# aslpavel/svgrasterize.py

Hardware: AMD Instinct MI355X
Metric: Mpixels/sec AA coverage+composite (path-pixels/s; whole step: flatten+binning+coverage+composite; planned replay -- a frame with new geometry: value_replan) (higher is better)
Workload: dtype f64 arithmetic, f32 RGBA store; 1 GPU; synthetic 4096 random closed cubic paths @ 4096x4096 (SURVEY 8d generator, splitmix64 0x5F3759DF); edges=783607

## Files before the change

### svgrasterize.py_amd/csrc/svgr_hip.hip

```cpp
#include <hip/hip_runtime.h>

#include <algorithm>
#include <atomic>
#include <cstdarg>
#include <cstddef>
#include <cmath>
#include <cstdio>
#include <cstring>
#include <ctime>
#include <initializer_list>
#include <new>
#include <string>
#include <type_traits>
#include <vector>
#include <memory>
#include <unordered_map>
#include <utility>

#include "../../include/svgr.h"
#include "svgr_core.h"

using namespace svgr;

static std::atomic<unsigned long long> g_n_launches{0};
// ... 493 lines not shown
    for (int k = 0; k < 2 * FL_ENDS; ++k) qe[k] = 0.0;
    constexpr int SEGL_ = 1 << SUB;
    if constexpr (PLACED) {
        int first = seg_ok ? lane_off[(size_t)seg * SEGL_ + sub] : 0;
        int nxt = __shfl_down(first, 1);
        if (sub == SEGL_ - 1) nxt = so1 - so0;
        const int n_plan = seg_ok ? nxt - first : 0;
        const int base_p = so0 + first;
        int n_found = 0;
        if (mode == 1) {
            track(node[0], node[1]);
            track(node[6], node[7]);
            n_found = 1;
            if (n_plan >= 1 && base_p < edge_cap) {
                store_edge(edges, base_p, node[0], node[1], node[6], node[7]);
                edge_path[base_p] = p;
            }
        } else if (mode == 2) {
            track(node[0], node[1]);
            int at = 0;
            n_found = flatten_subtree<1>(node, thr, kMaxFlattenDepth - SUB, [&](double r0_, double c0_, double r1, double c1) {
                track(r1, c1);
                if (at < n_plan && base_p + at < edge_cap) {
                    store_edge(edges, base_p + at, r0_, c0_, r1, c1);
                    edge_path[base_p + at] = p;
                }
                ++at;
            }, ovf);
        }
        if (ovf) atomicOr(&bd->err, 1);
        if (keep && n_found != n_plan) atomicOr(&bd->err, 2);
        if (seg_ok && sub == 0 && so1 > so0) atomicAdd(&bd->shard[(int)((blockIdx.x * (FL_BLOCK / 64) + (threadIdx.x >> 6)) % NSH)].cursor, so1 - so0);
    } else {
    const bool census = !EMIT && seg_cnt != nullptr;
    double rows_x = 0.0, cols_x = 0.0;
    if (mode == 1) {
        cnt = 1;
        track(node[0], node[1]);
        track(node[6], node[7]);
        if (census) { rows_x = fabs(node[6] - node[0]); cols_x = fabs(node[7] - node[1]); }
// ... 388 lines not shown
                    sl.e_begin = e_begin; sl.e_end = e_end; sl.pb_off = off;
                    sl.r0 = out[0]; sl.c0 = out[1]; sl.rows = out[2]; sl.cols = out[3];
                    sl.b0 = pb0; sl.cell_off = cell_off;
                    sl.pad[0] = sl.pad[1] = 0;
                    slabs[at++] = sl;
                }
            }
        }
    }
    if (p < n_paths) {
        ((int4*)bbox)[p] = make_int4(out[0], out[1], out[2], out[3]);
        PathBin pbin;
        pbin.b0 = pb0; pbin.nb = pnb; pbin.pb_off = off; pbin.cell_off = cell_off;
        bins[p] = pbin;
    }
}

__device__ __forceinline__ bool edge_prepare(const double* __restrict__ edges, const int* __restrict__ edge_path,
                                             const int* __restrict__ bbox, int e, EdgeSetup& es, int& p, int& r0) {
    p = edge_path[e];
    const int4 bb = ((const int4*)bbox)[p];
    r0 = bb.x;
    const int rows = bb.z, cols = bb.w;
    if (rows <= 0 || cols <= 0) return false;
    const double o_r = (double)bb.x, o_c = (double)bb.y;
    const double* ed = edges + 4 * (size_t)e;
    double ar = ed[0] - o_r, ac = ed[1] - o_c, br = ed[2] - o_r, bc = ed[3] - o_c;
    es = edge_setup(ar, ac, br, bc, rows);
    if (!es.valid) return false;
    double cmin = ac < bc ? ac : bc;
    if (cmin >= (double)cols + 2.0) return false;
    return true;
}

__device__ __forceinline__ void band_rows(const EdgeSetup& es, int band, int vr0, int r0, int& ya, int& yb) {
    const int b0row = band * TR + vr0 - r0;
    ya = es.y_begin > b0row ? es.y_begin : b0row;
    yb = es.y_end < b0row + TR ? es.y_end : b0row + TR;
}

struct TileEntry {
    int c0, cols;
    int cell0;
    int p;
    int r0, rows;
    int pad[2];
};
// ... 739 lines not shown
    int c = __popc(x);
    if (r >= c) { r -= c; pos = 32; x = (unsigned)(m >> 32); }
#pragma unroll
    for (int w = 16; w >= 1; w >>= 1) {
        const unsigned lo = x & ((1u << w) - 1u);
        c = __popc(lo);
        if (r >= c) { r -= c; pos += w; x >>= w; } else { x = lo; }
    }
    return pos;
}
__global__ __launch_bounds__(TL_BLOCK) void k_tile_lists(const int* __restrict__ band_start, const int* __restrict__ band_item0,
                                                         const TileEntry* __restrict__ entries, unsigned long long* __restrict__ tile_mask,
                                                         int mask_words, int n_ct, int vc0, Owner own, int n_owned,
                                                         int2* __restrict__ tile_info, uint4* __restrict__ pages,
                                                         uint4* __restrict__ items, const CellHdr* __restrict__ cell_hdr, int item_cap, int cell_cap,
                                                         BatchDev* __restrict__ bd, const PathBin* __restrict__ bins, const int* __restrict__ bbox) {
    constexpr int NWV = TL_BLOCK / 64;
    __shared__ int s_base[TL_BLOCK + 1], s_rank[TL_BLOCK];
    __shared__ int s_hist[64], s_cur[64], s_wtot[NWV];
    __shared__ int s_run;
    const int tid = threadIdx.x, lane = tid & 63, wave = tid >> 6;
    const int band = owned_band_at(own, blockIdx.x);
    const int W = mask_words;
    const int ent0 = band_start[band], item_band0 = band_item0[band];
    unsigned long long* const mband = tile_mask + (size_t)band * n_ct * 2 * W;
    auto count_tile = [&](int ct, int& n, int& n2) {
        n = 0; n2 = 0;
        const unsigned long long* mw = mband + (size_t)ct * 2 * W;
        for (int w = 0; w < W; ++w) { n += __popcll(mw[w]); n2 += __popcll(mw[W + w]); }
    };
    auto weight_of = [&](int n, int n2) { const int w = n + n2; return w < 63 ? w : 63; };
    if (tid < 64) s_hist[tid] = 0;
    if (tid == 0) s_run = 0;
    __syncthreads();
    const bool one_chunk = n_ct <= TL_BLOCK;
    int n_keep = 0, n2_keep = 0;
    for (int c0 = 0; c0 < n_ct; c0 += TL_BLOCK) {
        const int ct = c0 + tid;
        if (ct < n_ct) {
            int n, n2;
// ... 72 lines not shown
                const int4 eh = *(const int4*)(entries + ent0 + w * 64 + bit);
                cell = eh.z + tct - (eh.x - vc0) / TC;
            }
            const unsigned cls = ((mw[W + w] >> bit) & 1ull) ? 2u : 1u;
            cell = cell >= 0 && cell < cell_cap ? cell : 0;
            const long long at = (long long)item_band0 + run0 + i;
            const int4 hd = cls == 2u ? *(const int4*)((const char*)(cell_hdr + cell) + 48) : make_int4(0, 0, 0, 0);
            const uint4 it = make_uint4((unsigned)cell | (cls << 30), (unsigned)hd.z, (unsigned)hd.y, 0u);
            if (at < (long long)item_cap) items[at] = it;
            if (r_tile < PAGE_ITEMS) pages[((size_t)s_rank[lo] * n_owned + blockIdx.x) * PAGE_STRIDE + r_tile] = it;
        }
        __syncthreads();
        if (tid == 0) s_run = run0 + total;
        if (ct < n_ct) {
            unsigned long long* mw = mband + (size_t)ct * 2 * W;
            for (int w = 0; w < 2 * W; ++w) mw[w] = 0ull;
        }
        __syncthreads();
    }
}

constexpr int GRAD_MAX_STOPS = 32;
struct GradDev {
    int kind, spread, has_gt, n_stops;
    int excl_enabled, pad0, pad1, pad2;
    double user_m6[6], gt_m6[6];
    double p0[2], vec[2], vv;
    double center[2], radius;
    double fcenter[2], fradius, cd[2], rd, a, frad_rd, frad2, excl_thresh;
    double stop_off[GRAD_MAX_STOPS];
// ... 1963 lines not shown
    void wait_uploads() {
        if (up_pending && up_ev) (void)hipEventSynchronize(up_ev);
        up_pending = false;
        host_keep.clear();
    }
    DevArr<unsigned char> arena;
    size_t arena_bytes = 0, arena_laid = 0, off_pkeys = 0, off_prow = 0, off_scan = 0;
    DevArr<int> edge_path, bbox, band_start, band_count;
    DevArr<PathBin> bins;
    DevArr<TileEntry> entries;
    DevArr<double> edges;
    DevArr<CellHdr> cell_hdr;
    DevArr<unsigned char> work_block;
    DevArr<int2> cell_plan;
    bool add_places = false;
    void invalidate_work() { masks_zeroed = false; arena_zeroed = false; slabs_current = false; }
    DevArr<TileAdd> adds;
    DevArr<uint4> items;
    DevArr<int2> tile_info;
    DevArr<uint4> pages;
    DevArr<int> band_item0;
    AddShards add_shards{};
    int64_t n_adds = 0;
    bool count_adds_only = false;
    bool adds_roomy = false;
    bool fl_scan = false;
    bool late_scan = false;
    bool census_bbox = false;
    bool deterministic = false;
    int size_adds(const int* need, int n_shards) {
        if (int rc = layout_adds(need, n_shards)) return rc;
// ... 15 lines not shown
    DevArr<int> pair_idx;
    DevArr<Slab> slabs;
    DevArr<int> slab_at;
    bool slab_at_valid = false;
    bool slabs_current = false;
    bool slab_order_late = false;
    struct SlabsMade {
        const void *slabs, *bbox, *bins, *slab_at;
        int64_t n_slabs, n_paths;
        int vp[4];
        bool operator==(const SlabsMade& o) const {
            return slabs == o.slabs && bbox == o.bbox && bins == o.bins && slab_at == o.slab_at && n_slabs == o.n_slabs && n_paths == o.n_paths &&
                   vp[0] == o.vp[0] && vp[1] == o.vp[1] && vp[2] == o.vp[2] && vp[3] == o.vp[3];
        }
    } slabs_made{};
    bool slab_order_pending = false;
    std::vector<int> slab_at_host;
    int64_t n_slabs = 0;
    DevArr<int> seg_cnt, seg_off;
    int fl_sub = FL_SUB;
    DevArr<int> lane_off;
    DevArr<int> path_seg0;
    DevArr<int> seg_list;
    int64_t n_seg_list = -1;
    DevArr<int> path_list;
    int64_t n_path_list = 0;
    DevArr<unsigned long long> tile_mask;
    int mask_words = 1;
    bool masks_zeroed = false;
    DevArr<long long> layer_off;
    std::vector<long long> host_layer_off;
    bool geometry_fresh = false;
    bool geometry_current = false;
    bool arena_zeroed = false;
    int64_t n_edges_live = 0;
    int64_t n_edges = 0, n_pb = 0, n_bsegs = 0, n_cells = 0, n_entries = 0;
    int n_bands = 0;
    BatchDev host_bd{};
    EdgeShards shards{};
    std::vector<int> host_bbox;
    bool host_bbox_stale = false;
    bool defer_bbox = false;
    std::vector<TimedEvents> events;
    std::vector<hipEvent_t> event_pool;

    int n_ctiles() const { return (vp[3] + TC - 1) / TC; }
    int size_tile_lists(int owned_bands) {
        const size_t nt = (size_t)std::max(n_bands, 1) * (size_t)std::max(n_ctiles(), 1);
        if (int rc = tile_info.ensure(nt)) return rc;
        if (int rc = pages.ensure((size_t)std::max(owned_bands, 1) * (size_t)std::max(n_ctiles(), 1) * PAGE_STRIDE)) return rc;
        if (int rc = band_item0.ensure((size_t)n_bands + 1)) return rc;
        return items.ensure((size_t)std::max<int64_t>(n_cells, 1));
    }
    size_t mask_bytes() const { return sizeof(unsigned long long) * 2 * (size_t)mask_words * (size_t)n_bands * (size_t)n_ctiles(); }
    int size_masks(int64_t longest) {
        mask_words = (int)std::max<int64_t>((longest + 63) / 64, 1);
        masks_zeroed = false;
        return tile_mask.ensure(mask_bytes() / sizeof(unsigned long long) + 1);
    }
    bool census_set = false;
    BatchDev* bd() const { return (BatchDev*)arena.p + (census_set ? 1 : 0); }
    unsigned long long* pkeys() const { return (unsigned long long*)(arena.p + off_pkeys); }
    unsigned* prow() const { return (unsigned*)(arena.p + off_prow); }
    unsigned long long* scan_state() const { return (unsigned long long*)(arena.p + off_scan); }

    int layout_arena() {
        off_pkeys = 2 * sizeof(BatchDev);
        off_prow = off_pkeys + sizeof(unsigned long long) * 4 * (size_t)n_paths;
        off_scan = (off_prow + sizeof(unsigned) * 2 * (size_t)n_paths + 7) & ~(size_t)7;
        arena_bytes = off_scan + sizeof(unsigned long long) * (((size_t)n_segs << 6) / FL_BLOCK + 2);
        arena_bytes = (arena_bytes + 255) & ~(size_t)255;
        const unsigned char* const before = arena.p;
// ... 15 lines not shown
    int vp[4] = {0, 0, 0, 0};
    int64_t n_segs = 0, n_paths = 0;
    int mask_words = 1;
    AddShards add_shards{};
    int64_t n_adds = 0;
    bool adds_roomy = false;
    DevArr<int> edge_path, band_start, band_count, pair_idx, slab_at, seg_cnt, seg_off, lane_off, band_item0;
    DevArr<TileEntry> entries;
    DevArr<double> edges;
    DevArr<CellHdr> cell_hdr;
    DevArr<unsigned char> work_block;
    DevArr<int2> cell_plan, tile_info;
    DevArr<TileAdd> adds;
    DevArr<uint4> items, pages;
    DevArr<Slab> slabs;
    DevArr<unsigned long long> tile_mask;
};
#define SVGR_SPARE_ARRAYS(X) X(edge_path) X(band_start) X(band_count) X(pair_idx) X(slab_at) X(seg_cnt) X(seg_off) X(lane_off) X(band_item0) \
    X(entries) X(edges) X(cell_hdr) X(work_block) X(cell_plan) X(tile_info) X(adds) X(items) X(pages) X(slabs) X(tile_mask)
static void spare_stash(svgr_batch* b) {
    svgr_ctx* c = b->ctx;
    if (!b->sized || !b->has_vp || b->own.world > 1 || b->n_segs <= 4096 || !b->edges.p || !b->cell_plan.p || getenv("SVGR_NO_SPARE")) return;
    if (!c->spare) c->spare = new (std::nothrow) WorkSpare();
    if (!c->spare) return;
    WorkSpare& w = *c->spare;
    for (int k = 0; k < 4; ++k) w.vp[k] = b->sized_vp[k];
    w.n_segs = b->n_segs; w.n_paths = b->n_paths; w.mask_words = b->mask_words; w.add_shards = b->add_shards; w.n_adds = b->n_adds; w.adds_roomy = b->adds_roomy;
#define X(a) w.a = std::move(b->a);
    SVGR_SPARE_ARRAYS(X)
#undef X
}
static bool spare_adopt(svgr_batch* b) {
    svgr_ctx* c = b->ctx;
    WorkSpare* w = c->spare;
    if (!w || !w->edges.p || b->sized || !b->has_vp || b->own.world > 1 || b->n_segs <= 4096) return false;
    for (int k = 0; k < 4; ++k) if (w->vp[k] != b->vp[k]) return false;
    if (b->n_segs * 2 < w->n_segs || b->n_segs > w->n_segs + w->n_segs / 2 || b->n_paths * 2 < w->n_paths || b->n_paths > w->n_paths + w->n_paths / 2) return false;
    if (w->slab_at.cap && w->slab_at.cap < (size_t)b->n_paths) return false;
#define X(a) b->a = std::move(w->a);
    SVGR_SPARE_ARRAYS(X)
#undef X
    b->mask_words = w->mask_words; b->add_shards = w->add_shards; b->n_adds = w->n_adds; b->adds_roomy = w->adds_roomy;
    b->n_bands = (b->vp[2] + TR - 1) / TR;
    b->masks_zeroed = false;
    b->slab_at_valid = false; b->slabs_current = false;
    b->sized = true;
    for (int k = 0; k < 4; ++k) b->sized_vp[k] = b->vp[k];
    return true;
}

static inline dim3 grid1(size_t n, int block = 256) { return dim3((unsigned)((n + block - 1) / block)); }
static inline int cap_i32(size_t n) { return (int)std::min<size_t>(n, 0x7fffffff); }

static int choose_fl_sub(const svgr_batch* b, int n_items) {
    const size_t waves32 = ((size_t)std::max(n_items, 1) << 5) / 64, slots = (size_t)b->ctx->n_cu * 4 * 6;
    return waves32 * 2 <= slots ? 6 : 5;
}
static int run_geometry(svgr_batch* b, int upto, bool use_vp) {
    hipStream_t st = b->ctx->stream;
    const int ns = (int)b->n_segs, np = (int)b->n_paths;
    if (!b->arena_zeroed) HIPCHK(hipMemsetAsync(b->arena.p, 0, b->arena_bytes, st));
    b->arena_zeroed = false;
    const bool listed = use_vp && b->own.world > 1 && b->n_seg_list >= 0;
    const int n_items = listed ? (int)b->n_seg_list : ns;
    if (upto == 1) b->fl_sub = choose_fl_sub(b, n_items);
    const int fl_sub = b->fl_sub;
    const dim3 fgrid = grid1((size_t)std::max(n_items, 1) << fl_sub, FL_BLOCK);
    const int* seg_list = listed ? (const int*)b->seg_list.p : (const int*)nullptr;
    const int* plist = listed ? (const int*)b->path_list.p : (const int*)nullptr;
    const int np_walk = listed ? (int)b->n_path_list : np;
    const unsigned* prow = nullptr;
    if (use_vp && b->own.world > 1 && ns > 0 && !listed) {
        SVGR_LAUNCH(k_path_rows, grid1((size_t)ns), dim3(256), 0, st, (const double*)b->segs.p, (const uint8_t*)b->seg_kind.p,
                           (const int*)b->seg_path.p, (const double*)b->path_m6.p, ns, b->prow());
        prow = b->prow();
    }
    const int n_bands_vp = use_vp ? (b->vp[2] + TR - 1) / TR : 0;
// ... 6 lines not shown
        }
        if (ns > 0) {
            auto launch_cnt = [&](auto kern) {
                SVGR_LAUNCH(kern, fgrid, dim3(FL_BLOCK), 0, st, (const double*)b->segs.p,
                                   (const uint8_t*)b->seg_kind.p, (const int*)b->seg_path.p, (const double*)b->path_m6.p, ns,
                                   b->thr, (double*)nullptr, (int*)nullptr, b->shards, b->pkeys(), b->bd(), b->own, b->vp[0],
                                   n_bands_vp, prow, seg_list, n_items, upto == 1 ? b->seg_cnt.p : (int*)nullptr, (const int*)nullptr,
                                   use_vp ? b->vp[3] : 0 ,
                                   upto == 1 ? b->lane_off.p : (int*)nullptr, (int*)nullptr, (unsigned long long*)nullptr);
            };
            if (fl_sub == 6) launch_cnt(k_flatten<false, false, 6>); else launch_cnt(k_flatten<false, false, 5>);
        }
        if (upto == 1 && !b->late_scan)
            SVGR_LAUNCH(k_seg_scan, dim3(1), dim3(1024), 0, st, (const int*)b->seg_cnt.p, ns, b->seg_off.p);
        if (upto == 0 || (upto == 1 && b->census_bbox)) {
            b->slabs_current = false;
            SVGR_LAUNCH(k_path_bbox, grid1((size_t)std::max(np_walk, 1), 64), dim3(64), 0, st, (const unsigned long long*)b->pkeys(),
                               np_walk, use_vp ? 1 : 0, b->vp[0], b->vp[1], b->vp[2], b->vp[3], b->bbox.p, b->bins.p, b->bd(), 1, plist,
                               (Slab*)nullptr, 0, b->own, (const int*)nullptr, (const int*)nullptr, 0, (const int*)nullptr);
        }
        return 0;
    }
    if (ns > 0) {
        const bool lane_places = !b->safe_path;
        auto launch_fl = [&](auto kern, int* places) {
            SVGR_LAUNCH(kern, fgrid, dim3(FL_BLOCK), 0, st, (const double*)b->segs.p,
                               (const uint8_t*)b->seg_kind.p, (const int*)b->seg_path.p, (const double*)b->path_m6.p, ns, b->thr,
                               b->edges.p, b->edge_path.p, b->shards, b->pkeys(), b->bd(), b->own, b->vp[0],
                               n_bands_vp, prow, seg_list, n_items, (int*)nullptr, (const int*)b->seg_off.p,
                               cap_i32(std::min(b->edge_path.cap, b->edges.cap / 4)), places, (int*)nullptr, (unsigned long long*)nullptr);
        };
        const bool placed_fl = lane_places && b->lane_off.p && b->lane_off.cap >= ((size_t)ns << fl_sub);
        if (b->fl_scan) {
            auto launch_scan = [&](auto kern) {
                SVGR_LAUNCH(kern, fgrid, dim3(FL_BLOCK), 0, st, (const double*)b->segs.p,
                                   (const uint8_t*)b->seg_kind.p, (const int*)b->seg_path.p, (const double*)b->path_m6.p, ns, b->thr,
                                   b->edges.p, b->edge_path.p, b->shards, b->pkeys(), b->bd(), b->own, b->vp[0],
                                   n_bands_vp, prow, seg_list, n_items, b->seg_cnt.p, (const int*)nullptr,
                                   cap_i32(std::min(b->edge_path.cap, b->edges.cap / 4)), b->lane_off.p, b->seg_off.p, b->scan_state());
            };
            if (fl_sub == 6) launch_scan(k_flatten<true, false, 6, true>); else launch_scan(k_flatten<true, false, 5, true>);
        } else if (fl_sub == 6) {
            if (placed_fl) launch_fl(k_flatten<true, true, 6>, b->lane_off.p); else launch_fl(k_flatten<true, false, 6>, (int*)nullptr);
// ... 8 lines not shown
    const bool keep_slabs = slabs_for_plan && placed && b->slabs_current && b->slabs_made == slabs_now;
    if (!keep_slabs) {
        SVGR_LAUNCH(k_path_bbox, grid1((size_t)std::max(np_walk, 1), 64), dim3(64), 0, st, (const unsigned long long*)b->pkeys(), np_walk,
                           use_vp ? 1 : 0, b->vp[0], b->vp[1], b->vp[2], b->vp[3], b->bbox.p, b->bins.p, b->bd(), b->planned ? 0 : 1, plist,
                           upto >= 3 ? b->slabs.p : (Slab*)nullptr, (int)std::min<int64_t>(cap_i32(b->slabs.cap), b->n_slabs) , b->own,
                           (const int*)b->path_seg0.p, (const int*)b->seg_off.p,
                           cap_i32(std::min(b->edge_path.cap, b->edges.cap / 4)),
                           upto >= 4 && b->planned && b->slab_at_valid ? (const int*)b->slab_at.p : (const int*)nullptr);
        b->slabs_current = slabs_for_plan && !b->slab_order_late;
        b->slab_order_late = false;
        b->slabs_made = slabs_now;
    }
    if (upto == 2) return 0;
    const int owned = count_owned_bands(b->own, b->n_bands);
    const bool clear_in_be = owned > 0 && !keep_lists && upto >= 4 && !b->masks_zeroed && b->tile_mask.p && b->own.world <= 1;
    if (owned > 0 && !keep_lists)
        SVGR_LAUNCH(k_band_entries, dim3(owned), dim3(BE_BLOCK), 0, st, (const PathBin*)b->bins.p, np_walk, plist,
                           (const int*)b->bbox.p, b->band_start.p, b->band_count.p, b->band_item0.p, b->entries.p,
                           b->pair_idx.p, cap_i32(std::min(b->entries.cap, b->pair_idx.cap)),
                           upto >= 4 ? cap_i32(b->items.cap) : 0x7fffffff, b->vp[1], b->bd(), b->own,
                           upto >= 4 && b->planned && use_vp && !b->safe_path ? 1 : 0,
                           clear_in_be ? b->tile_mask.p : (unsigned long long*)nullptr, b->n_ctiles() * 2 * b->mask_words);
    if (clear_in_be) b->masks_zeroed = true;
    if (upto == 3) return 0;
    if (!b->masks_zeroed && b->tile_mask.p) {
        HIPCHK(hipMemsetAsync(b->tile_mask.p, 0, b->mask_bytes(), st));
        b->masks_zeroed = true;
    }
    unsigned long long* pb_dbg = nullptr;
#ifdef SVGR_DBG_PB_STAMP
    {
        static unsigned long long* buf = nullptr;
        if (!buf) { (void)hipMalloc((void**)&buf, 8 * 8 * 8192); (void)hipMemset(buf, 0, 8 * 8 * 8192); }
        pb_dbg = buf;
    }
#endif
    if (b->n_slabs > 0) {
        b->masks_zeroed = false;
        auto launch_pb = [&](auto kern) {
            SVGR_LAUNCH(kern, dim3((unsigned)b->n_slabs), dim3(PB_THREADS), 0, st, (const Slab*)b->slabs.p, (const double*)b->edges.p,
                               (const int*)b->pair_idx.p, (const double*)b->path_paint.p, (const uint8_t*)b->path_rule.p,
                               b->n_groups > 0 ? (const int*)b->path_group.p : (const int*)nullptr,
                               b->n_grads > 0 ? (const int*)b->path_grad.p : (const int*)nullptr, b->vp[0], b->vp[1], b->n_ctiles(), b->mask_words,
                               b->tile_mask.p, b->cell_hdr.p, cap_i32(std::min(b->cell_hdr.cap, b->cell_plan.cap)), b->add_shards,
                               b->count_adds_only ? (TileAdd*)nullptr : b->adds.p, b->cell_plan.p, b->bd(), b->own, b->planned ? 0 : 1,
                               b->deterministic ? 1 : 0, pb_dbg, keep_slabs ? (const unsigned long long*)b->pkeys() : (const unsigned long long*)nullptr,
                               (const int*)b->bbox.p, (const PathBin*)b->bins.p, np, b->vp[2], b->vp[3]);
        };
        const bool bounded = !placed && !b->count_adds_only && b->adds.p && b->adds_roomy && !b->safe_path && !getenv("SVGR_SAFE_PATH");
        if (getenv("SVGR_DBG_PLAN"))
            fprintf(stderr, "[geometry] k_path_build<%d>%s, %lld slabs, slab table %s\n", placed ? 1 : bounded ? 2 : 0,
                    b->count_adds_only ? " measuring" : "", (long long)b->n_slabs, keep_slabs ? "kept" : "written");
        if (placed) launch_pb(k_path_build<1>); else if (bounded) launch_pb(k_path_build<2>); else launch_pb(k_path_build<0>);
#ifdef SVGR_DBG_PB_STAMP
        if (pb_dbg && b->planned && !b->count_adds_only) {
            static int n_dump = 0;
            if (++n_dump == 20) {
                HIPCHK(hipStreamSynchronize(st));
                const size_t n = (size_t)std::min<int64_t>(b->n_slabs, 8192);
                std::vector<unsigned long long> h(8 * n);
                HIPCHK(hipMemcpy(h.data(), pb_dbg, sizeof(unsigned long long) * h.size(), hipMemcpyDeviceToHost));
                double ph[5] = {0, 0, 0, 0, 0}, rows_ = 0;
                unsigned long long lo = ~0ull, hi = 0;
                for (size_t i = 0; i < n; ++i) {
                    for (int q = 0; q < 5; ++q) ph[q] += (double)(h[8 * i + q + 1] - h[8 * i + q]);
                    rows_ += (double)h[8 * i + 6];
                    lo = std::min(lo, h[8 * i]); hi = std::max(hi, h[8 * i + 3]);
                }
                double s_rec = 0, s_edges = 0;
                for (size_t i = 0; i < n; ++i) { s_rec += (double)(h[8 * i + 7] - h[8 * i]); s_edges += (double)(h[8 * i + 5] - h[8 * i + 7]); }
                fprintf(stderr, "[pb stamp] %zu slabs, mean us: stage %.2f (slab record %.2f, edges landed +%.2f)  passA %.2f  walk %.2f | rows/slab %.0f | span %.1f us\n", n,
                        ph[0] / n / 100, s_rec / n / 100, s_edges / n / 100, ph[1] / n / 100, ph[2] / n / 100, rows_ / n, (double)(hi - lo) / 100);
                if (const char* f = getenv("SVGR_DBG_PB_DUMP")) { if (FILE* fp = fopen(f, "wb")) { fwrite(h.data(), 8, h.size(), fp); fclose(fp); } }
            }
        }
#endif
    }
    if (owned > 0 && b->n_ctiles() > 0) {
        SVGR_LAUNCH(k_tile_lists, dim3(owned), dim3(TL_BLOCK), 0, st, (const int*)b->band_start.p, (const int*)b->band_item0.p,
                           (const TileEntry*)b->entries.p, b->tile_mask.p, b->mask_words, b->n_ctiles(), b->vp[1], b->own, owned,
                           b->tile_info.p, b->pages.p, b->items.p, (const CellHdr*)b->cell_hdr.p, cap_i32(b->items.cap), cap_i32(b->cell_hdr.cap), b->bd(),
                           keep_lists ? (const PathBin*)b->bins.p : (const PathBin*)nullptr, (const int*)b->bbox.p);
        b->masks_zeroed = true;
    }
    return 0;
}

static int eval_dev_err(int e, int* capacity_bits) {
    if (capacity_bits) { *capacity_bits = e & (2 | 4 | 8 | 32 | 64); e &= ~(2 | 4 | 8 | 32 | 64); }
    if (e & 1) return fail(SVGR_E_OVERFLOW, "flatten depth cap (%d) hit: non-finite or absurd control points", kMaxFlattenDepth);
    if (e & 16) return fail(SVGR_E_INVALID, "path extent beyond +-1e9 pixels or non-finite");
    if (e & (2 | 4 | 8 | 32 | 64)) return fail(SVGR_E_OVERFLOW, "work buffer capacity exceeded (err bits %d): call svgr_batch_plan again", e);
    return 0;
}
static int issue_readback(svgr_batch* b, bool with_bboxes, void* staging = nullptr) {
    void* bd_dst = staging ? staging : (void*)&b->host_bd;
    HIPCHK(hipMemcpyAsync(bd_dst, b->bd(), sizeof(BatchDev), hipMemcpyDeviceToHost, b->ctx->stream));
    if (with_bboxes && !(b->defer_bbox && staging)) {
        b->host_bbox.resize(4 * (size_t)b->n_paths);
// ... 568 lines not shown

int svgr_batch_set_transforms(svgr_batch* b, const double* path_m6) {
    if (!b || !path_m6) return fail(SVGR_E_INVALID, "bad arguments");
    for (int64_t i = 0; i < 6 * b->n_paths; ++i)
        if (!std::isfinite(path_m6[i])) return fail(SVGR_E_INVALID, "non-finite transform");
    HIPCHK(enter_ctx(b->ctx));
    const size_t mbytes = sizeof(double) * 6 * (size_t)b->n_paths;
    if (void* hs = upload_stage(b->ctx, mbytes)) {
        memcpy(hs, path_m6, mbytes);
        HIPCHK(upload_staged(b->ctx, b->path_m6.p, mbytes));
    } else {
        b->wait_uploads();
        HIPCHK(hipMemcpyAsync(b->path_m6.p, b->keep(path_m6, mbytes), mbytes, hipMemcpyHostToDevice, b->ctx->stream));
        HIPCHK(b->note_upload(b->ctx->stream));
    }
    b->planned = false; b->slab_at_valid = false; b->slabs_current = false; b->slab_order_pending = false;
    return 0;
}

int svgr_batch_set_bands(svgr_batch* b, int rank, int world, int strip_bands) {
    if (!b || world <= 0 || rank < 0 || rank >= world || strip_bands <= 0) return fail(SVGR_E_INVALID, "bad band selection");
    b->own = Owner{rank, world, strip_bands};
    b->planned = false; b->slab_at_valid = false; b->slabs_current = false; b->slab_order_pending = false;
    b->sized = false;
    b->n_seg_list = -1;
    return 0;
}

int svgr_batch_set_groups(svgr_batch* b, const int32_t* path_group, int64_t n_groups, const int32_t* group_clip_src,
                          const double* group_opacity) {
    return abi_guard("svgr_batch_set_groups", [&]() -> int {
        if (!b) return fail(SVGR_E_INVALID, "batch is NULL");
        if (n_groups == 0) { b->n_groups = 0; b->geometry_fresh = false; b->geometry_current = false; return 0; }
        if (n_groups < 0 || n_groups > b->n_paths || !path_group || !group_clip_src || !group_opacity)
            return fail(SVGR_E_INVALID, "svgr_batch_set_groups: bad arguments");
        std::vector<int64_t> first((size_t)n_groups, -1), last((size_t)n_groups, -1);
        for (int64_t p = 0; p < b->n_paths; ++p) {
            const int g = path_group[p];
// ... 199 lines not shown
    return 1;
}
static int plan_slab_order(svgr_batch* b);
static int plan_speculative(svgr_batch* b) {
    for (int again = 1; again >= 0; --again) {
        const int is = spec_issue(b, nullptr, again != 0);
        if (is < 0) return is;
        if (is == 0) continue;
        HIPCHK(hipStreamSynchronize(b->ctx->stream));
        HIPCHK(hipGetLastError());
        const int fin = spec_finish(b);
        if (fin > 0 && b->n_segs > 4096) {
            if (int rc = plan_slab_order(b)) return rc;
        }
        if (fin != 0) return fin;
        b->planned = false; b->slabs_current = false;
    }
    return 0;
}

static int build_seg_list(svgr_batch* b) {
    hipStream_t st = b->ctx->stream;
    const int ns = (int)b->n_segs;
    if (int rc = b->seg_list.ensure((size_t)ns)) return rc;
    HIPCHK(hipMemsetAsync(b->arena.p, 0, b->arena_bytes, st));
    b->arena_zeroed = false;
    SVGR_LAUNCH(k_path_rows, grid1((size_t)ns), dim3(256), 0, st, (const double*)b->segs.p, (const uint8_t*)b->seg_kind.p,
                       (const int*)b->seg_path.p, (const double*)b->path_m6.p, ns, b->prow());
    SVGR_LAUNCH(k_seg_select, grid1((size_t)ns), dim3(256), 0, st, (const int*)b->seg_path.p, ns, (const unsigned*)b->prow(), b->own,
                       b->vp[0], (b->vp[2] + TR - 1) / TR, b->seg_list.p, &b->bd()->edge_spare);
    int n = 0;
// ... 48 lines not shown
        std::vector<char> issued((size_t)n, 0);
        std::vector<size_t> stage_off((size_t)n, 0);
        std::map<svgr_ctx*, size_t> stage_need;
        for (int64_t i = 0; i < n; ++i) {
            size_t& need = stage_need[batches[i]->ctx];
            stage_off[(size_t)i] = need;
            need += (sizeof(BatchDev) + 16 * (size_t)batches[i]->n_paths + 255) & ~(size_t)255;
        }
        for (auto& kv : stage_need) {
            HIPCHK(enter_ctx(kv.first));
            if (int rc = ensure_pinned(kv.first, kv.second)) return rc;
        }
        for (int64_t i = 0; i < n; ++i) {
            svgr_batch* b = batches[i];
            HIPCHK(enter_ctx(b->ctx));
            b->planned = false; b->slab_at_valid = false; b->slabs_current = false; b->slab_order_pending = false;
            b->geometry_fresh = false; b->geometry_current = false;
            const int is = no_spec ? 0 : spec_issue(b, (char*)b->ctx->pinned + stage_off[(size_t)i]);
            if (is < 0) return is;
            issued[(size_t)i] = (char)is;
        }
        for (int64_t i = 0; i < n; ++i)
            if (issued[(size_t)i]) {
                HIPCHK(enter_ctx(batches[i]->ctx));
                HIPCHK(hipStreamSynchronize(batches[i]->ctx->stream));
                HIPCHK(hipGetLastError());
                take_readback(batches[i], (const char*)batches[i]->ctx->pinned + stage_off[(size_t)i]);
            }
        for (int64_t i = 0; i < n; ++i) {
            svgr_batch* b = batches[i];
            int done = 0;
            if (issued[(size_t)i]) {
                done = spec_finish(b);
                if (done < 0) return done;
                if (done > 0 && b->n_segs > 4096)
                    if (int rc = plan_slab_order(b)) return rc;
            }
            if (!done)
                if (int rc = batch_plan_impl(b, issued[(size_t)i] != 0)) return rc;
        }
        return 0;
    });
}

static int plan_slab_order(svgr_batch* b) {
    b->slab_at_valid = false; b->slabs_current = false;
    b->slab_order_late = false;
    if (getenv("SVGR_SAFE_PATH")) return 0;
    const size_t np = (size_t)b->n_paths;
    if (int rc = ensure_host_bbox(b)) return rc;
    if (np == 0 || b->host_bbox.size() < 4 * np || b->n_slabs <= 0 || b->vp[2] <= 0) return 0;
    std::vector<int> n_sl(np, 0), order;
    std::vector<float> w(np, 0.f);
    order.reserve(np);
    long long total = 0;
    for (size_t p = 0; p < np; ++p) {
        const int r0 = b->host_bbox[4 * p], c0 = b->host_bbox[4 * p + 1], rows = b->host_bbox[4 * p + 2], cols = b->host_bbox[4 * p + 3];
        if (rows <= 0 || cols <= 0) continue;
        const int pb0 = (r0 - b->vp[0]) / TR, pnb = (r0 + rows - 1 - b->vp[0]) / TR - pb0 + 1;
        int ct0, pnct;
        path_ctiles(c0, cols, b->vp[1], ct0, pnct);
// ... 96 lines not shown
        diff[(size_t)b1 + 1] -= 1;
    }
    int longest = 0, run = 0;
    for (int k = 0; k < b->n_bands; ++k) { run += diff[(size_t)k]; longest = std::max(longest, run); }
    {
        double guess = 1.1 * (2.0 * (double)rows_x + (double)cols_x) + 14.0 * (double)b->n_cells + 65536.0;
        if (const char* sk = getenv("SVGR_TWO_PASS_SHRINK")) guess /= std::max(atof(sk), 1.0);
        if (guess > (double)(1ll << 29)) return 0;
        int need[NSH];
        for (int k = 0; k < NSH; ++k) need[k] = (int)(guess * 1.15 / NSH) + 8192;
        if ((rc = b->layout_adds(need, NSH))) return rc;
        b->adds_roomy = true;
    }
    b->mask_words = (int)std::max<int64_t>(((int64_t)std::max(longest, 1) + 63) / 64, 1);
    b->masks_zeroed = false;
    {
        const size_t n_e = (size_t)std::max<int64_t>(b->n_edges, 1), n_c = (size_t)std::max<int64_t>(b->n_cells, 1);
        const size_t n_pairs = (size_t)std::max<int64_t>(b->n_pb, 1), n_bd = (size_t)b->n_bands + 1;
        const size_t n_tiles = (size_t)std::max(b->n_bands, 1) * (size_t)std::max(b->n_ctiles(), 1);
        const size_t owned = (size_t)std::max(count_owned_bands(b->own, b->n_bands), 1);
        auto layout = [&](Carver& c) {
            c.take(b->edges, n_e * 4);
            c.take(b->edge_path, n_e);
            c.take(b->band_start, n_bd);
            c.take(b->band_count, n_bd);
            c.take(b->band_item0, n_bd);
            c.take(b->cell_hdr, n_c + 1);
            c.take(b->cell_plan, n_c + 1);
            c.take(b->slabs, (size_t)std::max<int64_t>(b->n_slabs, 1));
            c.take(b->entries, n_pairs);
            c.take(b->pair_idx, n_pairs);
            c.take(b->tile_mask, b->mask_bytes() / sizeof(unsigned long long) + 1);
            c.take(b->tile_info, n_tiles);
            c.take(b->pages, owned * (size_t)std::max(b->n_ctiles(), 1) * PAGE_STRIDE);
            c.take(b->items, n_c);
            c.take(b->adds, (size_t)std::max<int64_t>(b->n_adds, 1));
        };
        Carver sizing;
        layout(sizing);
        b->edges.release(); b->edge_path.release(); b->band_start.release(); b->band_count.release(); b->band_item0.release();
        b->cell_hdr.release(); b->cell_plan.release(); b->slabs.release(); b->entries.release(); b->pair_idx.release();
        b->tile_mask.release(); b->tile_info.release(); b->pages.release(); b->items.release(); b->adds.release();
        b->work_block.release();
        if ((rc = b->work_block.ensure(sizing.at))) return rc;
        Carver carve;
        carve.base = b->work_block.p;
        layout(carve);
    }
    const double t_3 = now_ms();
    if ((rc = run_geometry(b, 4, true))) return rc;
    if ((rc = issue_readback(b, staging == nullptr, staging))) return rc;
    if (getenv("SVGR_DBG_PLAN"))
        fprintf(stderr, "[plan] two passes, ms: pass 1 issued %.3f, drained %.3f, buffers sized %.3f, pass 2 issued %.3f | edges %lld, rows crossed %lld, columns %lld, pairs %lld, cells %lld, slabs %lld, add slots %lld, longest band list %d\n",
                t_1 - t_0, t_2 - t_1, t_3 - t_2, now_ms() - t_3, n_edges, rows_x, cols_x, (long long)b->n_pb, (long long)b->n_cells, (long long)b->n_slabs, (long long)b->n_adds, longest);
    return 1;
}
static int two_pass_finish(svgr_batch* b, const void* staging) {
// ... 21 lines not shown

static int plan_two_pass(svgr_batch* b) {
    const int is = two_pass_issue(b, nullptr);
    if (is <= 0) return is;
    HIPCHK(hipStreamSynchronize(b->ctx->stream));
    const int fin = two_pass_finish(b, nullptr);
    if (fin <= 0) return fin;
    if (int rc = plan_slab_order(b)) return rc;
    return 1;
}

static int batch_plan_impl(svgr_batch* b, bool skip_speculative) {
    if (!b) return fail(SVGR_E_INVALID, "batch is NULL");
    HIPCHK(enter_ctx(b->ctx));
    b->defer_bbox = false;
    b->planned = false; b->slab_at_valid = false; b->slabs_current = false; b->slab_order_pending = false;
    b->geometry_fresh = false; b->geometry_current = false;
    {
        const bool no_spec = getenv("SVGR_NO_SPECULATIVE_PLAN") != nullptr;
        const int sp = no_spec || skip_speculative ? 0 : plan_speculative(b);
        if (sp < 0) return sp;
        if (sp > 0) return 0;
    }
    {
        const int tp = plan_two_pass(b);
        if (tp < 0) return tp;
        if (tp > 0) return 0;
        b->planned = false; b->slab_at_valid = false; b->slabs_current = false; b->slab_order_pending = false;
        b->geometry_fresh = false; b->geometry_current = false;
    }
    if (int rc = b->layout_arena()) return rc;
    if (!b->has_vp) {
        if (int rc = run_geometry(b, 0, false)) return rc;
        if (int rc = check_dev_err(b)) return rc;
        if (b->host_bd.n_nonempty > 0) {
            long long r0 = (long long)UNION_BIAS - (long long)b->host_bd.umin_r, c0 = (long long)UNION_BIAS - (long long)b->host_bd.umin_c;
            long long ur = (long long)b->host_bd.umax_r - UNION_BIAS - r0, uc = (long long)b->host_bd.umax_c - UNION_BIAS - c0;
            if (ur * uc > (1ll << 31) || ur > (1 << 24) || uc > (1 << 24))
                return fail(SVGR_E_INVALID, "unclipped extent of %lldx%lld pixels is too large; pass a viewport", ur, uc);
            b->vp[0] = (int)r0; b->vp[1] = (int)c0; b->vp[2] = (int)ur; b->vp[3] = (int)uc;
        } else {
            b->vp[0] = b->vp[1] = 0; b->vp[2] = b->vp[3] = 0;
        }
// ... 423 lines not shown
}

static int batch_draw_impl(svgr_batch* b, svgr_buf* out, int out_kind, unsigned flags) {
    if (!b || !out) return fail(SVGR_E_INVALID, "bad arguments");
    HIPCHK(enter_ctx(b->ctx));
    hipStream_t st = b->ctx->stream;
    b->defer_bbox = false;
    if (!b->planned) {
        const bool canvas = out_kind == SVGR_OUT_CANVAS_F32 || out_kind == SVGR_OUT_CANVAS_F64;
        const bool fast = canvas && b->has_vp && b->own.world <= 1 && b->n_segs > 0 && !(flags & (SVGR_RENDER_TIMED | SVGR_RENDER_DETERMINISTIC)) &&
                          getenv("SVGR_NO_SPECULATIVE_PLAN") == nullptr && getenv("SVGR_SAFE_PATH") == nullptr;
        int issued = 0;
        if (fast) {
            const size_t stage_bytes = sizeof(BatchDev) + 16 * (size_t)b->n_paths + 256;
            if (int rc = ensure_pinned(b->ctx, stage_bytes)) return rc;
            b->slab_at_valid = false; b->slabs_current = false; b->slab_order_pending = false;
            b->geometry_fresh = false; b->geometry_current = false;
            b->defer_bbox = true;
            int is = spec_issue(b, b->ctx->pinned, true);
            b->defer_bbox = is > 0;
            if (is == 0) is = spec_issue(b, b->ctx->pinned, false);
            if (is < 0) return is;
            if (is > 0) issued = 1;
            else {
                is = two_pass_issue(b, b->ctx->pinned);
                if (is < 0) return is;
                if (is > 0) issued = 2;
            }
        }
        if (issued) {
            b->planned = true; b->geometry_fresh = true; b->geometry_current = true;
            int rc = batch_render_impl(b, out, out_kind, flags, nullptr);
            b->planned = false; b->slabs_current = false; b->geometry_fresh = false; b->geometry_current = false;
            hipError_t e = hipStreamSynchronize(st);
            if (rc) return rc;
            HIPCHK(e);
            int fin;
            if (issued == 1) { take_readback(b, b->ctx->pinned); HIPCHK(hipGetLastError()); fin = spec_finish(b); }
            else fin = two_pass_finish(b, b->ctx->pinned);
            b->defer_bbox = false;
            if (fin < 0) return fin;
            if (fin > 0) {
                b->geometry_fresh = false;
                b->slab_order_pending = b->n_segs > 4096;
                return 0;
            }
            b->planned = false; b->slab_at_valid = false; b->slabs_current = false; b->slab_order_pending = false;
        }
        if (int rc = batch_plan_impl(b, issued == 1)) return rc;
    }
    if (int rc = batch_render_impl(b, out, out_kind, flags, nullptr)) return rc;
    HIPCHK(hipStreamSynchronize(st));
    return check_dev_err(b, nullptr, false);
}
int svgr_batch_draw(svgr_batch* b, svgr_buf* out, int out_kind, unsigned flags) {
    return abi_guard("svgr_batch_draw", [&]() { return batch_draw_impl(b, out, out_kind, flags); });
}

int svgr_batch_timings(svgr_batch* b, int* n_renders, double* ms_total, double* ms_geometry, double* ms_tile) {
    if (!b) return fail(SVGR_E_INVALID, "batch is NULL");
    HIPCHK(enter_ctx(b->ctx));
    HIPCHK(hipStreamSynchronize(b->ctx->stream));
// ... 1767 lines not shown
```

Before: 811,400 Mpixels/s.

## Reuse tile lists when tile masks are unchanged across planned replays

```diff
diff --git a/svgrasterize.py_amd/csrc/svgr_hip.hip b/svgrasterize.py_amd/csrc/svgr_hip.hip
--- a/svgrasterize.py_amd/csrc/svgr_hip.hip
+++ b/svgrasterize.py_amd/csrc/svgr_hip.hip
@@ -531,7 +531,7 @@
             n_found = 1;
             if (n_plan >= 1 && base_p < edge_cap) {
                 store_edge(edges, base_p, node[0], node[1], node[6], node[7]);
-                edge_path[base_p] = p;
+                if (edge_path) edge_path[base_p] = p;
             }
         } else if (mode == 2) {
             track(node[0], node[1]);
@@ -540,7 +540,7 @@
                 track(r1, c1);
                 if (at < n_plan && base_p + at < edge_cap) {
                     store_edge(edges, base_p + at, r0_, c0_, r1, c1);
-                    edge_path[base_p + at] = p;
+                    if (edge_path) edge_path[base_p + at] = p;
                 }
                 ++at;
             }, ovf);
@@ -959,23 +959,6 @@
         pbin.b0 = pb0; pbin.nb = pnb; pbin.pb_off = off; pbin.cell_off = cell_off;
         bins[p] = pbin;
     }
-}
-
-__device__ __forceinline__ bool edge_prepare(const double* __restrict__ edges, const int* __restrict__ edge_path,
-                                             const int* __restrict__ bbox, int e, EdgeSetup& es, int& p, int& r0) {
-    p = edge_path[e];
-    const int4 bb = ((const int4*)bbox)[p];
-    r0 = bb.x;
-    const int rows = bb.z, cols = bb.w;
-    if (rows <= 0 || cols <= 0) return false;
-    const double o_r = (double)bb.x, o_c = (double)bb.y;
-    const double* ed = edges + 4 * (size_t)e;
-    double ar = ed[0] - o_r, ac = ed[1] - o_c, br = ed[2] - o_r, bc = ed[3] - o_c;
-    es = edge_setup(ar, ac, br, bc, rows);
-    if (!es.valid) return false;
-    double cmin = ac < bc ? ac : bc;
-    if (cmin >= (double)cols + 2.0) return false;
-    return true;
 }
 
 __device__ __forceinline__ void band_rows(const EdgeSetup& es, int band, int vr0, int r0, int& ya, int& yb) {
@@ -1745,7 +1728,8 @@
                                                          int mask_words, int n_ct, int vc0, Owner own, int n_owned,
                                                          int2* __restrict__ tile_info, uint4* __restrict__ pages,
                                                          uint4* __restrict__ items, const CellHdr* __restrict__ cell_hdr, int item_cap, int cell_cap,
-                                                         BatchDev* __restrict__ bd, const PathBin* __restrict__ bins, const int* __restrict__ bbox) {
+                                                         BatchDev* __restrict__ bd, const PathBin* __restrict__ bins, const int* __restrict__ bbox,
+                                                         unsigned long long* __restrict__ tile_mask_kept, int kept) {
     constexpr int NWV = TL_BLOCK / 64;
     __shared__ int s_base[TL_BLOCK + 1], s_rank[TL_BLOCK];
     __shared__ int s_hist[64], s_cur[64], s_wtot[NWV];
@@ -1753,8 +1737,44 @@
     const int tid = threadIdx.x, lane = tid & 63, wave = tid >> 6;
     const int band = owned_band_at(own, blockIdx.x);
     const int W = mask_words;
+    unsigned long long* const mband = tile_mask + (size_t)band * n_ct * 2 * W;
+    unsigned long long* const kband = tile_mask_kept ? tile_mask_kept + (size_t)band * n_ct * 2 * W : nullptr;
+    if (kept) {
+        __shared__ int s_wdiff[NWV];
+        auto any_differs = [&](bool d) {
+            const bool wd = __ballot(d) != 0ull;
+            if (lane == 0) s_wdiff[wave] = wd ? 1 : 0;
+            __syncthreads();
+            int a = 0;
+#pragma unroll
+            for (int w = 0; w < NWV; ++w) a |= s_wdiff[w];
+            return a != 0;
+        };
+        unsigned long long diff = 0ull;
+        if (W == 1 && n_ct <= TL_BLOCK) {
+            ulonglong2 m = make_ulonglong2(0ull, 0ull), k = m;
+            if (tid < n_ct) { m = ((const ulonglong2*)mband)[tid]; k = ((const ulonglong2*)kband)[tid]; }
+            diff = (m.x ^ k.x) | (m.y ^ k.y);
+            if (!any_differs(diff != 0ull)) {
+                if ((m.x | m.y) != 0ull) ((ulonglong2*)mband)[tid] = make_ulonglong2(0ull, 0ull);
+                return;
+            }
+        } else {
+            for (int ct = tid; ct < n_ct; ct += TL_BLOCK) {
+                const unsigned long long* mw = mband + (size_t)ct * 2 * W;
+                const unsigned long long* kw = kband + (size_t)ct * 2 * W;
+                for (int w = 0; w < 2 * W; ++w) diff |= mw[w] ^ kw[w];
+            }
+            if (!any_differs(diff != 0ull)) {
+                for (int ct = tid; ct < n_ct; ct += TL_BLOCK) {
+                    unsigned long long* mw = mband + (size_t)ct * 2 * W;
+                    for (int w = 0; w < 2 * W; ++w) mw[w] = 0ull;
+                }
+                return;
+            }
+        }
+    }
     const int ent0 = band_start[band], item_band0 = band_item0[band];
-    unsigned long long* const mband = tile_mask + (size_t)band * n_ct * 2 * W;
     auto count_tile = [&](int ct, int& n, int& n2) {
         n = 0; n2 = 0;
         const unsigned long long* mw = mband + (size_t)ct * 2 * W;
@@ -1857,6 +1877,10 @@
         if (tid == 0) s_run = run0 + total;
         if (ct < n_ct) {
             unsigned long long* mw = mband + (size_t)ct * 2 * W;
+            if (kband) {
+                unsigned long long* kw = kband + (size_t)ct * 2 * W;
+                for (int w = 0; w < 2 * W; ++w) kw[w] = mw[w];
+            }
             for (int w = 0; w < 2 * W; ++w) mw[w] = 0ull;
         }
         __syncthreads();
@@ -3850,7 +3874,7 @@
     DevArr<unsigned char> work_block;
     DevArr<int2> cell_plan;
     bool add_places = false;
-    void invalidate_work() { masks_zeroed = false; arena_zeroed = false; slabs_current = false; }
+    void invalidate_work() { masks_zeroed = false; arena_zeroed = false; slabs_current = false; lists_current = false; }
     DevArr<TileAdd> adds;
     DevArr<uint4> items;
     DevArr<int2> tile_info;
@@ -3896,6 +3920,22 @@
                    vp[0] == o.vp[0] && vp[1] == o.vp[1] && vp[2] == o.vp[2] && vp[3] == o.vp[3];
         }
     } slabs_made{};
+    bool lists_current = false;
+    struct ListsMade {
+        const void *items, *pages, *tile_info, *entries, *bins, *bbox, *cell_hdr, *cell_plan, *tile_mask, *tile_mask_kept;
+        size_t items_cap, pages_cap, tile_info_cap, entries_cap, bins_cap, bbox_cap, cell_hdr_cap, cell_plan_cap, tile_mask_cap, tile_mask_kept_cap;
+        int n_ctiles, mask_words, owned;
+        int vp[4];
+        bool operator==(const ListsMade& o) const {
+            return items == o.items && pages == o.pages && tile_info == o.tile_info && entries == o.entries && bins == o.bins && bbox == o.bbox &&
+                   cell_hdr == o.cell_hdr && cell_plan == o.cell_plan && tile_mask == o.tile_mask && tile_mask_kept == o.tile_mask_kept &&
+                   items_cap == o.items_cap && pages_cap == o.pages_cap && tile_info_cap == o.tile_info_cap && entries_cap == o.entries_cap &&
+                   bins_cap == o.bins_cap && bbox_cap == o.bbox_cap && cell_hdr_cap == o.cell_hdr_cap && cell_plan_cap == o.cell_plan_cap &&
+                   tile_mask_cap == o.tile_mask_cap && tile_mask_kept_cap == o.tile_mask_kept_cap && n_ctiles == o.n_ctiles &&
+                   mask_words == o.mask_words && owned == o.owned && vp[0] == o.vp[0] && vp[1] == o.vp[1] && vp[2] == o.vp[2] && vp[3] == o.vp[3];
+        }
+    } lists_made{};
+    unsigned long long stale_word = 0ull;
     bool slab_order_pending = false;
     std::vector<int> slab_at_host;
     int64_t n_slabs = 0;
@@ -3908,6 +3948,7 @@
     DevArr<int> path_list;
     int64_t n_path_list = 0;
     DevArr<unsigned long long> tile_mask;
+    DevArr<unsigned long long> tile_mask_kept;
     int mask_words = 1;
     bool masks_zeroed = false;
     DevArr<long long> layer_off;
@@ -3938,6 +3979,8 @@
     int size_masks(int64_t longest) {
         mask_words = (int)std::max<int64_t>((longest + 63) / 64, 1);
         masks_zeroed = false;
+        lists_current = false;
+        if (int rc = tile_mask_kept.ensure(mask_bytes() / sizeof(unsigned long long) + 1)) return rc;
         return tile_mask.ensure(mask_bytes() / sizeof(unsigned long long) + 1);
     }
     bool census_set = false;
@@ -3983,10 +4026,10 @@
     DevArr<TileAdd> adds;
     DevArr<uint4> items, pages;
     DevArr<Slab> slabs;
-    DevArr<unsigned long long> tile_mask;
+    DevArr<unsigned long long> tile_mask, tile_mask_kept;
 };
 #define SVGR_SPARE_ARRAYS(X) X(edge_path) X(band_start) X(band_count) X(pair_idx) X(slab_at) X(seg_cnt) X(seg_off) X(lane_off) X(band_item0) \
-    X(entries) X(edges) X(cell_hdr) X(work_block) X(cell_plan) X(tile_info) X(adds) X(items) X(pages) X(slabs) X(tile_mask)
+    X(entries) X(edges) X(cell_hdr) X(work_block) X(cell_plan) X(tile_info) X(adds) X(items) X(pages) X(slabs) X(tile_mask) X(tile_mask_kept)
 static void spare_stash(svgr_batch* b) {
     svgr_ctx* c = b->ctx;
     if (!b->sized || !b->has_vp || b->own.world > 1 || b->n_segs <= 4096 || !b->edges.p || !b->cell_plan.p || getenv("SVGR_NO_SPARE")) return;
@@ -4012,7 +4055,7 @@
     b->mask_words = w->mask_words; b->add_shards = w->add_shards; b->n_adds = w->n_adds; b->adds_roomy = w->adds_roomy;
     b->n_bands = (b->vp[2] + TR - 1) / TR;
     b->masks_zeroed = false;
-    b->slab_at_valid = false; b->slabs_current = false;
+    b->slab_at_valid = false; b->slabs_current = false; b->lists_current = false;
     b->sized = true;
     for (int k = 0; k < 4; ++k) b->sized_vp[k] = b->vp[k];
     return true;
@@ -4030,6 +4073,7 @@
     const int ns = (int)b->n_segs, np = (int)b->n_paths;
     if (!b->arena_zeroed) HIPCHK(hipMemsetAsync(b->arena.p, 0, b->arena_bytes, st));
     b->arena_zeroed = false;
+    if (upto < 4) b->lists_current = false;
     const bool listed = use_vp && b->own.world > 1 && b->n_seg_list >= 0;
     const int n_items = listed ? (int)b->n_seg_list : ns;
     if (upto == 1) b->fl_sub = choose_fl_sub(b, n_items);
@@ -4066,7 +4110,7 @@
         if (upto == 1 && !b->late_scan)
             SVGR_LAUNCH(k_seg_scan, dim3(1), dim3(1024), 0, st, (const int*)b->seg_cnt.p, ns, b->seg_off.p);
         if (upto == 0 || (upto == 1 && b->census_bbox)) {
-            b->slabs_current = false;
+            b->slabs_current = false; b->lists_current = false;
             SVGR_LAUNCH(k_path_bbox, grid1((size_t)std::max(np_walk, 1), 64), dim3(64), 0, st, (const unsigned long long*)b->pkeys(),
                                np_walk, use_vp ? 1 : 0, b->vp[0], b->vp[1], b->vp[2], b->vp[3], b->bbox.p, b->bins.p, b->bd(), 1, plist,
                                (Slab*)nullptr, 0, b->own, (const int*)nullptr, (const int*)nullptr, 0, (const int*)nullptr);
@@ -4075,10 +4119,11 @@
     }
     if (ns > 0) {
         const bool lane_places = !b->safe_path;
+        const bool keep_edge_path = b->planned && lane_places && b->lane_off.p && b->lane_off.cap >= ((size_t)ns << fl_sub) && !b->fl_scan;
         auto launch_fl = [&](auto kern, int* places) {
             SVGR_LAUNCH(kern, fgrid, dim3(FL_BLOCK), 0, st, (const double*)b->segs.p,
                                (const uint8_t*)b->seg_kind.p, (const int*)b->seg_path.p, (const double*)b->path_m6.p, ns, b->thr,
-                               b->edges.p, b->edge_path.p, b->shards, b->pkeys(), b->bd(), b->own, b->vp[0],
+                               b->edges.p, keep_edge_path ? (int*)nullptr : b->edge_path.p, b->shards, b->pkeys(), b->bd(), b->own, b->vp[0],
                                n_bands_vp, prow, seg_list, n_items, (int*)nullptr, (const int*)b->seg_off.p,
                                cap_i32(std::min(b->edge_path.cap, b->edges.cap / 4)), places, (int*)nullptr, (unsigned long long*)nullptr);
         };
@@ -4117,6 +4162,7 @@
     if (upto == 2) return 0;
     const int owned = count_owned_bands(b->own, b->n_bands);
     const bool clear_in_be = owned > 0 && !keep_lists && upto >= 4 && !b->masks_zeroed && b->tile_mask.p && b->own.world <= 1;
+    if (!keep_lists) b->lists_current = false;
     if (owned > 0 && !keep_lists)
         SVGR_LAUNCH(k_band_entries, dim3(owned), dim3(BE_BLOCK), 0, st, (const PathBin*)b->bins.p, np_walk, plist,
                            (const int*)b->bbox.p, b->band_start.p, b->band_count.p, b->band_item0.p, b->entries.p,
@@ -4138,6 +4184,14 @@
         pb_dbg = buf;
     }
 #endif
+    const size_t mask_n = b->mask_bytes() / sizeof(unsigned long long);
+    const bool lists_for_plan = slabs_for_plan && placed && owned > 0 && b->n_ctiles() > 0 && b->tile_mask.p && b->tile_mask_kept.p &&
+                                b->tile_mask.cap >= mask_n && b->tile_mask_kept.cap >= mask_n;
+    const svgr_batch::ListsMade lists_now{b->items.p, b->pages.p, b->tile_info.p, b->entries.p, b->bins.p, b->bbox.p, b->cell_hdr.p, b->cell_plan.p,
+                                          b->tile_mask.p, b->tile_mask_kept.p, b->items.cap, b->pages.cap, b->tile_info.cap, b->entries.cap,
+                                          b->bins.cap, b->bbox.cap, b->cell_hdr.cap, b->cell_plan.cap, b->tile_mask.cap, b->tile_mask_kept.cap,
+                                          b->n_ctiles(), b->mask_words, owned, {b->vp[0], b->vp[1], b->vp[2], b->vp[3]}};
+    const bool lists_kept = lists_for_plan && keep_slabs && b->lists_current && b->lists_made == lists_now;
     if (b->n_slabs > 0) {
         b->masks_zeroed = false;
         auto launch_pb = [&](auto kern) {
@@ -4152,8 +4206,10 @@
         };
         const bool bounded = !placed && !b->count_adds_only && b->adds.p && b->adds_roomy && !b->safe_path && !getenv("SVGR_SAFE_PATH");
         if (getenv("SVGR_DBG_PLAN"))
-            fprintf(stderr, "[geometry] k_path_build<%d>%s, %lld slabs, slab table %s\n", placed ? 1 : bounded ? 2 : 0,
-                    b->count_adds_only ? " measuring" : "", (long long)b->n_slabs, keep_slabs ? "kept" : "written");
+            fprintf(stderr, "[geometry] k_path_build<%d>%s, %lld slabs, tile lists %s, slab table %s\n", placed ? 1 : bounded ? 2 : 0,
+                    b->count_adds_only ? " measuring" : "", (long long)b->n_slabs,
+                    lists_kept ? "kept" : "rebuilt" ,
+                    keep_slabs ? "kept" : "written");
         if (placed) launch_pb(k_path_build<1>); else if (bounded) launch_pb(k_path_build<2>); else launch_pb(k_path_build<0>);
 #ifdef SVGR_DBG_PB_STAMP
         if (pb_dbg && b->planned && !b->count_adds_only) {
@@ -4180,12 +4236,26 @@
 #endif
     }
     if (owned > 0 && b->n_ctiles() > 0) {
+        if (lists_kept)
+            if (const char* sb = getenv("SVGR_DBG_STALE_BAND")) {
+                const int band = atoi(sb);
+                if (band >= 0 && band < b->n_bands) {
+                    unsigned long long* const w0 = b->tile_mask_kept.p + (size_t)band * b->n_ctiles() * 2 * b->mask_words;
+                    HIPCHK(hipMemcpyAsync(&b->stale_word, w0, sizeof(unsigned long long), hipMemcpyDeviceToHost, st));
+                    HIPCHK(hipStreamSynchronize(st));
+                    b->stale_word ^= 1ull;
+                    HIPCHK(hipMemcpyAsync(w0, &b->stale_word, sizeof(unsigned long long), hipMemcpyHostToDevice, st));
+                }
+            }
         SVGR_LAUNCH(k_tile_lists, dim3(owned), dim3(TL_BLOCK), 0, st, (const int*)b->band_start.p, (const int*)b->band_item0.p,
                            (const TileEntry*)b->entries.p, b->tile_mask.p, b->mask_words, b->n_ctiles(), b->vp[1], b->own, owned,
                            b->tile_info.p, b->pages.p, b->items.p, (const CellHdr*)b->cell_hdr.p, cap_i32(b->items.cap), cap_i32(b->cell_hdr.cap), b->bd(),
-                           keep_lists ? (const PathBin*)b->bins.p : (const PathBin*)nullptr, (const int*)b->bbox.p);
+                           keep_lists ? (const PathBin*)b->bins.p : (const PathBin*)nullptr, (const int*)b->bbox.p,
+                           lists_for_plan ? b->tile_mask_kept.p : (unsigned long long*)nullptr, lists_kept ? 1 : 0);
         b->masks_zeroed = true;
     }
+    b->lists_current = lists_for_plan;
+    b->lists_made = lists_now;
     return 0;
 }
 
@@ -4784,14 +4854,14 @@
         HIPCHK(hipMemcpyAsync(b->path_m6.p, b->keep(path_m6, mbytes), mbytes, hipMemcpyHostToDevice, b->ctx->stream));
         HIPCHK(b->note_upload(b->ctx->stream));
     }
-    b->planned = false; b->slab_at_valid = false; b->slabs_current = false; b->slab_order_pending = false;
+    b->planned = false; b->slab_at_valid = false; b->slabs_current = false; b->lists_current = false; b->slab_order_pending = false;
     return 0;
 }
 
 int svgr_batch_set_bands(svgr_batch* b, int rank, int world, int strip_bands) {
     if (!b || world <= 0 || rank < 0 || rank >= world || strip_bands <= 0) return fail(SVGR_E_INVALID, "bad band selection");
     b->own = Owner{rank, world, strip_bands};
-    b->planned = false; b->slab_at_valid = false; b->slabs_current = false; b->slab_order_pending = false;
+    b->planned = false; b->slab_at_valid = false; b->slabs_current = false; b->lists_current = false; b->slab_order_pending = false;
     b->sized = false;
     b->n_seg_list = -1;
     return 0;
@@ -5021,7 +5091,7 @@
             if (int rc = plan_slab_order(b)) return rc;
         }
         if (fin != 0) return fin;
-        b->planned = false; b->slabs_current = false;
+        b->planned = false; b->slabs_current = false; b->lists_current = false;
     }
     return 0;
 }
@@ -5100,7 +5170,7 @@
         for (int64_t i = 0; i < n; ++i) {
             svgr_batch* b = batches[i];
             HIPCHK(enter_ctx(b->ctx));
-            b->planned = false; b->slab_at_valid = false; b->slabs_current = false; b->slab_order_pending = false;
+            b->planned = false; b->slab_at_valid = false; b->slabs_current = false; b->lists_current = false; b->slab_order_pending = false;
             b->geometry_fresh = false; b->geometry_current = false;
             const int is = no_spec ? 0 : spec_issue(b, (char*)b->ctx->pinned + stage_off[(size_t)i]);
             if (is < 0) return is;
@@ -5130,7 +5200,7 @@
 }
 
 static int plan_slab_order(svgr_batch* b) {
-    b->slab_at_valid = false; b->slabs_current = false;
+    b->slab_at_valid = false; b->slabs_current = false; b->lists_current = false;
     b->slab_order_late = false;
     if (getenv("SVGR_SAFE_PATH")) return 0;
     const size_t np = (size_t)b->n_paths;
@@ -5257,6 +5327,7 @@
     }
     b->mask_words = (int)std::max<int64_t>(((int64_t)std::max(longest, 1) + 63) / 64, 1);
     b->masks_zeroed = false;
+    b->lists_current = false;
     {
         const size_t n_e = (size_t)std::max<int64_t>(b->n_edges, 1), n_c = (size_t)std::max<int64_t>(b->n_cells, 1);
         const size_t n_pairs = (size_t)std::max<int64_t>(b->n_pb, 1), n_bd = (size_t)b->n_bands + 1;
@@ -5274,6 +5345,7 @@
             c.take(b->entries, n_pairs);
             c.take(b->pair_idx, n_pairs);
             c.take(b->tile_mask, b->mask_bytes() / sizeof(unsigned long long) + 1);
+            c.take(b->tile_mask_kept, b->mask_bytes() / sizeof(unsigned long long) + 1);
             c.take(b->tile_info, n_tiles);
             c.take(b->pages, owned * (size_t)std::max(b->n_ctiles(), 1) * PAGE_STRIDE);
             c.take(b->items, n_c);
@@ -5283,7 +5355,7 @@
         layout(sizing);
         b->edges.release(); b->edge_path.release(); b->band_start.release(); b->band_count.release(); b->band_item0.release();
         b->cell_hdr.release(); b->cell_plan.release(); b->slabs.release(); b->entries.release(); b->pair_idx.release();
-        b->tile_mask.release(); b->tile_info.release(); b->pages.release(); b->items.release(); b->adds.release();
+        b->tile_mask.release(); b->tile_mask_kept.release(); b->tile_info.release(); b->pages.release(); b->items.release(); b->adds.release();
         b->work_block.release();
         if ((rc = b->work_block.ensure(sizing.at))) return rc;
         Carver carve;
@@ -5335,7 +5407,7 @@
     if (!b) return fail(SVGR_E_INVALID, "batch is NULL");
     HIPCHK(enter_ctx(b->ctx));
     b->defer_bbox = false;
-    b->planned = false; b->slab_at_valid = false; b->slabs_current = false; b->slab_order_pending = false;
+    b->planned = false; b->slab_at_valid = false; b->slabs_current = false; b->lists_current = false; b->slab_order_pending = false;
     b->geometry_fresh = false; b->geometry_current = false;
     {
         const bool no_spec = getenv("SVGR_NO_SPECULATIVE_PLAN") != nullptr;
@@ -5347,7 +5419,7 @@
         const int tp = plan_two_pass(b);
         if (tp < 0) return tp;
         if (tp > 0) return 0;
-        b->planned = false; b->slab_at_valid = false; b->slabs_current = false; b->slab_order_pending = false;
+        b->planned = false; b->slab_at_valid = false; b->slabs_current = false; b->lists_current = false; b->slab_order_pending = false;
         b->geometry_fresh = false; b->geometry_current = false;
     }
     if (int rc = b->layout_arena()) return rc;
@@ -5801,7 +5873,7 @@
         if (fast) {
             const size_t stage_bytes = sizeof(BatchDev) + 16 * (size_t)b->n_paths + 256;
             if (int rc = ensure_pinned(b->ctx, stage_bytes)) return rc;
-            b->slab_at_valid = false; b->slabs_current = false; b->slab_order_pending = false;
+            b->slab_at_valid = false; b->slabs_current = false; b->lists_current = false; b->slab_order_pending = false;
             b->geometry_fresh = false; b->geometry_current = false;
             b->defer_bbox = true;
             int is = spec_issue(b, b->ctx->pinned, true);
@@ -5818,7 +5890,7 @@
         if (issued) {
             b->planned = true; b->geometry_fresh = true; b->geometry_current = true;
             int rc = batch_render_impl(b, out, out_kind, flags, nullptr);
-            b->planned = false; b->slabs_current = false; b->geometry_fresh = false; b->geometry_current = false;
+            b->planned = false; b->slabs_current = false; b->lists_current = false; b->geometry_fresh = false; b->geometry_current = false;
             hipError_t e = hipStreamSynchronize(st);
             if (rc) return rc;
             HIPCHK(e);
@@ -5832,7 +5904,7 @@
                 b->slab_order_pending = b->n_segs > 4096;
                 return 0;
             }
-            b->planned = false; b->slab_at_valid = false; b->slabs_current = false; b->slab_order_pending = false;
+            b->planned = false; b->slab_at_valid = false; b->slabs_current = false; b->lists_current = false; b->slab_order_pending = false;
         }
         if (int rc = batch_plan_impl(b, issued == 1)) return rc;
     }
```

New measurement: 836,800 Mpixels/s (median of 6 runs). 3.1% higher.
